# nicolaivicol/otto-recommender

Hardware: AMD Instinct MI355X
Metric: co-visit pairs/sec + candidates/sec at 220M events, 1/2/4/8 MI355X (higher is better)
Workload: dtype int32; 1 GPU; configs[1]: all 5 co-visitation rules, 220M events, 100k-session files; events=220000079, sessions=13435907, parallelism=files dealt over 1 GPU(s)

## Files before the change

### otto-recommender_amd/csrc/abi.hip

```cpp
#include <cstdarg>
#include <cstdlib>
#include <ctime>
#include <algorithm>
#include <mutex>
#include "prims.h"
#include "covis_kernels.h"
#include "table.h"

using namespace ottohip;

namespace ottohip {
static thread_local char g_err[1024] = "";
void set_error(const char* fmt, ...) {
  va_list ap;
  va_start(ap, fmt);
  vsnprintf(g_err, sizeof g_err, fmt, ap);
  va_end(ap);
}
}

namespace ottohip {
Ctx* ctx_base(ottohip_ctx* c) { return c; }

int ensure_part_stats(const ottohip_table* tc) {
// ... 96 lines not shown
  const int dev = it->second.first;
  auto& fr = g_cache[dev].free_;
  fr.emplace(it->second.second, p);
  g_cache_live.erase(it);
  size_t tot = 0;
  for (auto& kv : fr) tot += kv.first;
  if (tot <= cache_cap()) return;
  int prev = -1;
  (void)hipGetDevice(&prev);
  if (prev != dev) (void)hipSetDevice(dev);
  while (tot > cache_cap() && !fr.empty()) {
    auto last = std::prev(fr.end());
    tot -= last->first;
    (void)hipDeviceSynchronize();
    (void)hipFree(last->second);
    fr.erase(last);
  }
  if (prev != dev) (void)hipSetDevice(prev);
}

void dev_trim() {
  std::lock_guard<std::mutex> lk(g_cache_mu);
  auto it = g_cache.find(cur_device());
  if (it == g_cache.end() || it->second.free_.empty()) return;
  (void)hipDeviceSynchronize();
  for (auto& kv : it->second.free_) (void)hipFree(kv.second);
  it->second.free_.clear();
}
}


struct Front {
  RulesDev R;
  Layout Lt;
  int64_t E = 0, Sn = 0, NB = 0;
  int nl = 0;
  const int64_t* off = nullptr;
  int64_t *first = nullptr, *fb = nullptr, *d_loff = nullptr;
  int32_t* long_list = nullptr;
  uint32_t* fid = nullptr;
  uint64_t* evp = nullptr;
  uint64_t* lscr = nullptr;
  uint32_t* lpscr = nullptr;
  uint32_t* cnt = nullptr;
  uint32_t* link = nullptr;
  uint64_t* poff = nullptr;
  uint32_t* poff32 = nullptr;
  uint64_t P = 0;
  int64_t Rn = 0;
  uint32_t* row_key = nullptr;
  uint64_t* row_begin = nullptr;
};

struct KeptEmission {
  uint32_t* words = nullptr;
  uint32_t* row_key = nullptr;
  uint64_t* row_begin = nullptr;
  uint64_t P = 0;
  int64_t Rn = 0;
  RulesDev R;
  Layout Lt;
  int n_rules = 0, n_files = 0;
};
void kept_free(KeptEmission* k) {
  if (!k) return;
  dev_free(k->words);
// ... 71 lines not shown
static ottohip_table* new_table(ottohip_ctx* ctx, int n_rules, int32_t n_items) {
  ottohip_table* T = new ottohip_table();
  T->device = ctx->device;
  T->n_rules = n_rules;
  T->n_items = n_items;
  T->ctx = ctx;
  memset(T->stats, 0, sizeof T->stats);
  return T;
}

static int owner_map(ottohip_ctx* ctx, int32_t n_items, int G, hipStream_t s, const uint32_t** a2l,
                     const uint32_t** l2a, const uint32_t** obase, int* LB) {
  uint32_t *da2l, *dl2a, *dob;
  OH_TRY(ctx->ws.get("om_a2l", (size_t)std::max(n_items, 1), &da2l));
  OH_TRY(ctx->ws.get("om_l2a", (size_t)std::max(n_items, 1), &dl2a));
  OH_TRY(ctx->ws.get("om_obase", (size_t)G + 1, &dob));
  if (ctx->om_items != n_items || ctx->om_parts != G) {
    std::vector<uint32_t> cnt(G + 1, 0), a2l_h(std::max(n_items, 1)), l2a_h(std::max(n_items, 1));
    for (int32_t a = 0; a < n_items; ++a) a2l_h[a] = cnt[owner_dev((uint32_t)a, (uint32_t)G)]++;
    uint32_t mx = 0;
    std::vector<uint32_t> ob(G + 1, 0);
    for (int o = 0; o < G; ++o) { mx = std::max(mx, cnt[o]); ob[o + 1] = ob[o] + cnt[o]; }
    for (int32_t a = 0; a < n_items; ++a) l2a_h[ob[owner_dev((uint32_t)a, (uint32_t)G)] + a2l_h[a]] = (uint32_t)a;
    OH_HIP(hipMemcpyAsync(da2l, a2l_h.data(), (size_t)n_items * 4, hipMemcpyHostToDevice, s));
    OH_HIP(hipMemcpyAsync(dl2a, l2a_h.data(), (size_t)n_items * 4, hipMemcpyHostToDevice, s));
    OH_HIP(hipMemcpyAsync(dob, ob.data(), (size_t)(G + 1) * 4, hipMemcpyHostToDevice, s));
    OH_HIP(hipStreamSynchronize(s));
    ctx->om_items = n_items;
    ctx->om_parts = G;
    ctx->om_lb = std::max(1, bits_for((uint64_t)mx));
  }
  *a2l = da2l; *l2a = dl2a; *obase = dob; *LB = ctx->om_lb;
  return 0;
}

static int covis_front(ottohip_ctx* ctx, const ottohip_events* ev, const ottohip_covis_params* params,
                       const int32_t* file_ids, int n_parts, Front& F, hipStream_t s, ottohip_emit* EM = nullptr) {
  ++ctx->gen;
  const int64_t E = ev->n_events, Sn = ev->n_sessions;
  F.E = E; F.Sn = Sn;
  F.P = 0; F.Rn = 0;
  if (E == 0 || Sn == 0) return 0;
  Workspace& ws = ctx->ws;
  const Layout& Lt = F.Lt;
  const RulesDev& R = F.R;
  const int64_t NB = ceil_div(E, EV_BLOCK);
  F.NB = NB;
  int32_t* n_long;
  int* err;
  const int64_t long_cap = E / (LCAP + 1) + 1;
  OH_TRY(ws.get("first", (size_t)NB + 1, &F.first));
  OH_TRY(ws.get("fb", (size_t)ev->n_files + 1, &F.fb));
  OH_TRY(ws.get("fid", (size_t)ev->n_files, &F.fid));
  OH_TRY(ws.get("long_list", (size_t)long_cap, &F.long_list));
  OH_TRY(ws.get("n_long", 4, &n_long));
  OH_TRY(ws.get("err", 4, &err));
  std::vector<uint32_t> fid(ev->n_files);
  for (int f = 0; f < ev->n_files; ++f) fid[f] = file_ids ? (uint32_t)file_ids[f] : (uint32_t)f;
  OH_HIP(hipMemcpyAsync(F.fb, ev->file_session_bounds, (ev->n_files + 1) * sizeof(int64_t), hipMemcpyHostToDevice, s));
  OH_HIP(hipMemcpyAsync(F.fid, fid.data(), ev->n_files * sizeof(uint32_t), hipMemcpyHostToDevice, s));
  OH_HIP(hipMemsetAsync(n_long, 0, 4 * sizeof(int32_t), s));
  OH_HIP(hipMemsetAsync(err, 0, sizeof(int), s));
  OH_HIP(hipStreamSynchronize(s));
  const int64_t* off = ev->session_offsets;
  F.off = off;

  uint32_t *rk, *pos, *rk2, *pos2;
  OH_TRY(ws.get("ev", (size_t)E, &F.evp));
  OH_TRY(ws.get("cnt", (size_t)E, &F.cnt));
  OH_TRY(ws.get("rk", (size_t)E, &rk));
  OH_TRY(ws.get("pos", (size_t)E, &pos));
  OH_TRY(ws.get("rk2", (size_t)E, &rk2));
  OH_TRY(ws.get("pos2", (size_t)E, &pos2));
  static const bool rows_legacy = getenv("OTTOHIP_ROWS") && !strcmp(getenv("OTTOHIP_ROWS"), "legacy");
  const int cshift = (Lt.A + 2 + 7) / 8 * 8;
  const bool ol_env = !(getenv("OTTOHIP_OWNER_LOCAL") && !strcmp(getenv("OTTOHIP_OWNER_LOCAL"), "0"));
  const uint32_t *om_a2l = nullptr, *om_l2a = nullptr, *om_obase = nullptr;
  int om_lb = 0;
  bool owner_local = false;
  if (!rows_legacy && n_parts > 1 && ol_env && cshift + 8 <= 32 && 3ull * (uint64_t)params->n_items < (1ull << 24)) {
    OH_TRY(owner_map(ctx, params->n_items, n_parts, s, &om_a2l, &om_l2a, &om_obase, &om_lb));
    owner_local = ((uint64_t)n_parts << (om_lb + 2)) < (1ull << cshift);
  }
  const bool fused = !rows_legacy && (n_parts == 1 || owner_local) && cshift + 8 <= 32 &&
                     3ull * (uint64_t)params->n_items < (1ull << 24);
  uint32_t* pos_w = fused ? nullptr : pos;
  static const bool rows_atomic = getenv("OTTOHIP_ROWS") && !strcmp(getenv("OTTOHIP_ROWS"), "atomic");
  const bool group = fused && !rows_atomic && !(getenv("OTTOHIP_GROUP") && !strcmp(getenv("OTTOHIP_GROUP"), "0"));
  F.link = nullptr;
  if (group) OH_TRY(ws.get("link", (size_t)E, &F.link));
  int ph = ctx->begin("prep_count", s, 9.0 * E + 8.0 * (Sn + 1) + 8.0 * E + 12.0 * E);
  k_block_first<<<grid_for(Sn + 1), 256, 0, s>>>(off, Sn, NB, F.first, F.long_list, n_long);
  k_prep_count<<<(unsigned)NB, 64, 0, s>>>(off, F.first, NB, ev->aid, ev->ts, ev->type, F.evp, params->n_items,
                                           params->dedup, err, R, Lt.A, F.cnt, rk, pos_w, fused ? cshift : 0, F.link);
  if (hipGetLastError() != hipSuccess) { set_error("k_prep_count launch failed"); return OTTOHIP_EHIP; }
  int32_t nl = 0;
  OH_TRY(d2h(&nl, n_long, 1, s));
  F.nl = nl;
  if (nl > 0) {
    std::vector<int32_t> ll(nl);
    OH_TRY(d2h(ll.data(), F.long_list, (size_t)nl, s));
    std::sort(ll.begin(), ll.end());
    OH_HIP(hipMemcpy(F.long_list, ll.data(), nl * sizeof(int32_t), hipMemcpyHostToDevice));
    std::vector<int64_t> loff(nl + 1);
    loff[0] = 0;
    for (int i = 0; i < nl; ++i) {
      int64_t ab[2];
      OH_HIP(hipMemcpy(ab, off + ll[i], 2 * sizeof(int64_t), hipMemcpyDeviceToHost));
      loff[i + 1] = loff[i] + (ab[1] - ab[0]);
    }
    OH_TRY(ws.get("long_scr", (size_t)(2 * loff[nl]), &F.lscr));
    OH_TRY(ws.get("long_pscr", (size_t)(3 * (loff[nl] + nl)), &F.lpscr));
    OH_TRY(ws.get("long_off", (size_t)(nl + 1), &F.d_loff));
    OH_HIP(hipMemcpy(F.d_loff, loff.data(), (nl + 1) * sizeof(int64_t), hipMemcpyHostToDevice));
    k_prep_long<<<nl, 64, 0, s>>>(off, F.long_list, F.d_loff, F.lscr, ev->aid, ev->ts, ev->type, F.evp,
                                  params->n_items, params->dedup, err);
    k_count_long<<<nl, 64, 0, s>>>(off, F.long_list, F.d_loff, F.lscr, F.lpscr, F.evp, R, Lt.A, F.cnt, rk, pos_w,
                                   fused ? cshift : 0, F.link);
    if (hipGetLastError() != hipSuccess) { set_error("long-session launch failed"); return OTTOHIP_EHIP; }
  }
  ctx->end(ph, s);

  ph = ctx->begin("rows", s, 0);
  if (rows_atomic && fused) {
    const uint32_t INVa = 3u << Lt.A;
    const uint32_t kmask_a = Lt.A + 2 >= 32 ? ~0u : (1u << (Lt.A + 2)) - 1u;
    const int64_t nk = (int64_t)3 << Lt.A;
// ... 103 lines not shown
  uint64_t *woff, *row_idx;
  OH_TRY(ws.get("woff", (size_t)E, &woff));
  OH_TRY(ws.get("row_idx", (size_t)E, &row_idx));
  OH_TRY(exclusive_scan_u32(ctx, c_sorted, woff, E, tot, s));
  OH_TRY(exclusive_scan_u32(ctx, row_flag, row_idx, E, tot + 1, s));
  uint64_t PR[2];
  OH_TRY(d2h(PR, tot, 2, s));
  int herr = 0;
  OH_TRY(d2h(&herr, err, 1, s));
  if (herr) { set_error("input out of range: aid outside [0, n_items) or type outside {0,1,2}"); return OTTOHIP_ERANGE; }
  F.P = PR[0];
  F.Rn = (int64_t)PR[1];
  OH_TRY(ws.get("poff", (size_t)E, &F.poff));
  F.poff32 = nullptr;
  OH_TRY(ws.get("row_key", (size_t)std::max<int64_t>(F.Rn, 1), &F.row_key));
  OH_TRY(ws.get("row_begin", (size_t)std::max<int64_t>(F.Rn, 1), &F.row_begin));
  k_rows<<<grid_for(E), 256, 0, s>>>(rks, poss, E, INV, kmask, woff, row_flag, row_idx, F.poff, F.row_key,
                                     F.row_begin);
  ctx->end(ph, s);
  return 0;
}

static int covis_emit_words(ottohip_ctx* ctx, const Front& F, const ottohip_events* ev, uint32_t* w0, hipStream_t s) {
  int ph = ctx->begin("emit", s, 8.0 * F.E + 12.0 * F.E + 4.0 * (double)F.P);
  static const int dbg0 = getenv("OTTOHIP_EMIT_DBG") ? atoi(getenv("OTTOHIP_EMIT_DBG")) : 0;
  const int dbg = dbg0;
  const bool guard = getenv("OTTOHIP_DEBUG") != nullptr;
  int* eerr;
  OH_TRY(ctx->ws.get("emit_err", 4, &eerr));
  OH_HIP(hipMemsetAsync(eerr, 0, sizeof(int), s));
  const bool tasks = !(getenv("OTTOHIP_EMIT_TASKS") && !strcmp(getenv("OTTOHIP_EMIT_TASKS"), "0"));
  const bool fl2 = !(getenv("OTTOHIP_EMIT_FLUSH2") && !strcmp(getenv("OTTOHIP_EMIT_FLUSH2"), "0"));
  const bool flq = tasks && fl2 && !(getenv("OTTOHIP_EMIT_FLUSHQ") && !strcmp(getenv("OTTOHIP_EMIT_FLUSHQ"), "0"));
  auto ek = guard ? (tasks ? (flq ? k_emit<true, true, true, EB_Q> : k_emit<true, true, true>) : k_emit<true, false, true>)
                  : (tasks ? (flq ? k_emit<false, true, true, EB_Q> : fl2 ? k_emit<false, true, true> : k_emit<false, true, false>)
                           : k_emit<false, false, true>);
  if (F.NB > 0)
    ek<<<(unsigned)F.NB, 64, 0, s>>>(F.off, F.first, F.NB, F.evp, F.R, F.Lt, F.fb, ev->n_files, F.fid, F.cnt,
                                         EvOff{F.poff, F.poff32, nullptr}, w0, eerr, dbg);
  if (F.nl > 0)
    k_emit_long<<<F.nl, 64, 0, s>>>(F.off, F.long_list, F.d_loff, F.lscr, F.lpscr, F.evp, F.R, F.Lt, F.fb,
                                     ev->n_files, F.fid, F.cnt, EvOff{F.poff, F.poff32, nullptr}, w0);
  if (hipGetLastError() != hipSuccess) { set_error("k_emit launch failed"); return OTTOHIP_EHIP; }
  ctx->end(ph, s);
  int herr = 0;
  OH_TRY(d2h(&herr, eerr, 1, s));
  if (herr & 8) { set_error("emit: record index outside the flush's records (err=%d)", herr); return OTTOHIP_EHIP; }
  if (herr) { set_error("emit: pairs written per event disagree with the count stage (err=%d)", herr); return OTTOHIP_EHIP; }
  return 0;
}

static int file_opts_setup(ottohip_ctx* ctx, const ottohip_file_opts* o, int n_rules, const RulesDev& R,
                           FileOpts& fo, hipStream_t s) {
  if (o->rule < 0 || o->rule >= n_rules) { set_error("file_opts: rule %d outside the call's rules", o->rule); return OTTOHIP_EINVAL; }
  const bool want_hist = o->file_rows || o->file_rows_ge2;
  if (want_hist && (o->n_files < 1 || o->n_files > FO_MAXF)) {
    set_error("file_opts: n_files=%d outside [1, %d]", o->n_files, FO_MAXF); return OTTOHIP_ELIMIT;
  }
  memset(&fo, 0, sizeof fo);
  for (int t = 0; t < 3; ++t)
    for (int q = 0; q < R.n_of_type[t]; ++q)
      if (R.rule_of_type[t][q] == o->rule) { fo.type = t; fo.q = (uint32_t)q; }
  fo.sym = (uint32_t)((R.sym_mask >> o->rule) & 1u);
  if (fo.sym && (o->lo_file >= 0 || o->hi_file >= 0)) { set_error("file_opts: key cuts on a symmetric table"); return OTTOHIP_EINVAL; }
  fo.lo_file = o->lo_file < 0 ? 0xFFFFFFFFu : (uint32_t)o->lo_file;
  fo.hi_file = o->hi_file < 0 ? 0xFFFFFFFFu : (uint32_t)o->hi_file;
  fo.cuts = (o->lo_file >= 0 || o->hi_file >= 0) ? 1u : 0u;
  fo.lo_key = o->lo_key;
  fo.hi_key = o->hi_key;
  OH_TRY(ctx->ws.get("fo_dropped", 1, &fo.dropped));
  OH_HIP(hipMemsetAsync(fo.dropped, 0, 8, s));
  if (getenv("OTTOHIP_DEBUG")) {
// ... 1456 lines not shown
```

### otto-recommender_amd/csrc/covis_kernels.h

```cpp
#pragma once
#include "prims.h"

namespace ottohip {

constexpr int EV_BLOCK = 256;
constexpr int LCAP = 512;
constexpr int SPLIT_MEAN = 420;
constexpr int LDS_SPLIT_MEAN = 2560;
__constant__ uint32_t c_split_mean = SPLIT_MEAN;
__constant__ uint32_t c_split_runs = 0;
__constant__ uint32_t c_split_fuse = 1;
__constant__ uint32_t c_hash_prio = 0;
__constant__ uint32_t c_lds_leaf = 0;
constexpr uint32_t W_EMPTY = 0xFFFFFFFFu;
constexpr int STAT_STRIPES = 256;
constexpr int STAT_RAW = MAX_RULES * 4;
constexpr int STAT_STRIDE = STAT_RAW + 8;

struct RulesDev {
  int32_t lo[MAX_RULES], hi[MAX_RULES];
  uint32_t mask[MAX_RULES];
  int32_t n_of_type[4];
  int32_t rule_of_type[4][MAX_RULES];
  uint32_t sym_mask;
};

__device__ __forceinline__ bool rule_sym(const RulesDev& R, int r) { return (R.sym_mask >> r) & 1u; }

__device__ __forceinline__ uint32_t count_sym_partners(const uint64_t* ev, int jb, int je, uint32_t aid, int t, int A) {
  const uint32_t lo = (aid << 2) | (uint32_t)t;
  uint32_t m = 0;
  if (A > 29) {
    for (int j = jb; j < je; ++j) {
      const uint32_t w = (uint32_t)ev[j];
      m += ((w & 3u) == (uint32_t)t && w >= lo) ? 1u : 0u;
    }
    return m;
  }
  constexpr uint32_t LIM = 1u << 29;
  auto ok = [&](uint32_t w) { return __builtin_amdgcn_alignbit(w - lo, w - lo, 2) < LIM ? 1u : 0u; };
  int j = jb;
  for (; j + 4 <= je; j += 4) m += ok((uint32_t)ev[j]) + ok((uint32_t)ev[j + 1]) + ok((uint32_t)ev[j + 2]) + ok((uint32_t)ev[j + 3]);
  for (; j < je; ++j) m += ok((uint32_t)ev[j]);
  return m;
}

struct Layout {
  int A;
  int F;
  int BR;
  int WB;
  uint32_t amask;
};

struct Task {
  uint64_t begin;
  uint32_t len;
  uint32_t row;
  uint32_t rem;
  uint32_t buf;
// ... 253 lines not shown
                                                   uint32_t* __restrict__ pos, int cshift, uint32_t* __restrict__ link) {
  const int64_t s = list[blockIdx.x];
  const int64_t e0 = off[s];
  const int n = (int)(off[s + 1] - e0);
  const int64_t so = scratch_off[blockIdx.x];
  SessView S;
  uint64_t* evs = scratch + 2 * so;
  uint32_t* pref = pscratch + 3 * (so + blockIdx.x);
  S.ev = evs; S.pref = pref; S.pstride = n + 1;
  S.nv = load_session(ev + e0, n, evs, pref, n + 1);
  count_session(S, e0, n, R, A, cnt, rk, pos, cshift, link);
}

__device__ __forceinline__ int lds_lower_ts(const uint64_t* tev, int a, int b, int64_t x) {
  while (a < b) {
    const int m = (a + b) >> 1;
    if ((int64_t)ev_ts(tev[m]) < x) a = m + 1; else b = m;
  }
  return a;
}
__device__ __forceinline__ int lds_upper_ts(const uint64_t* tev, int a, int b, int64_t x) {
  while (a < b) {
    const int m = (a + b) >> 1;
    if ((int64_t)ev_ts(tev[m]) <= x) a = m + 1; else b = m;
  }
  return a;
}

constexpr int PB_CAP = 512;
struct PrepLds {
  uint64_t key[PB_CAP];
  union {
    uint64_t srt[PB_CAP];
    uint16_t pref[3][PB_CAP + 1];
  };
  uint16_t ss[65];
  uint16_t pst[64], pen[64];
  uint8_t esid[PB_CAP];
  uint8_t uns[64];
};
static_assert((uint64_t)PB_CAP * MAX_RULES * (LCAP - 1) < (1ull << LK_DSHIFT), "group prefixes in link bits");

__global__ __launch_bounds__(64) void k_prep_count(const int64_t* __restrict__ off, const int64_t* __restrict__ first,
                                                   int64_t NB, const int32_t* __restrict__ aid,
                                                   const int32_t* __restrict__ ts, const int8_t* __restrict__ ty,
                                                   uint64_t* __restrict__ ev, int n_items, int dedup, int* err,
                                                   RulesDev R, int A, uint32_t* __restrict__ cnt,
                                                   uint32_t* __restrict__ rk, uint32_t* __restrict__ pos, int cshift,
                                                   uint32_t* __restrict__ link) {
  __shared__ PrepLds S;
  __shared__ RulesDev sR;
  const int l = threadIdx.x;
  if (l == 0) sR = R;
  const int64_t g = blockIdx.x;
  if (g >= NB) return;
  const int64_t s0 = first[g], s1 = first[g + 1];
  __syncthreads();
  const uint32_t INV = 3u << A;
  int64_t b = s0;
  while (b < s1) {
    const int64_t base = off[b];
    const int64_t s = b + l;
    const bool in_s = s < s1;
    const int64_t so = in_s ? off[s] : 0, se = in_s ? off[s + 1] : 0;
    const bool ok = in_s && se - base <= PB_CAP && se - so <= LCAP;
    const uint64_t bad = __ballot(!ok);
    const int nsess = bad ? (int)__builtin_ctzll(bad) : 64;
    if (nsess == 0) { ++b; continue; }
    const int nb_ev = __shfl((int)(se - base), nsess - 1);
    const int64_t E0 = base;
    if (l < nsess) { S.ss[l] = (uint16_t)(so - base); S.uns[l] = 0; }
    if (l == 0) S.ss[nsess] = (uint16_t)nb_ev;
    __builtin_amdgcn_wave_barrier();
    __builtin_amdgcn_fence(__ATOMIC_SEQ_CST, "wavefront");
    const int nch = (nb_ev + 63) >> 6;
#pragma unroll 1
    for (int c = 0; c < nch; ++c) {
      const int idx = c * 64 + l;
      if (idx >= nb_ev) continue;
      const int32_t a = aid[E0 + idx], t = ts[E0 + idx], y = ty[E0 + idx];
      if (a < 0 || a >= n_items || y < 0 || y > 2) atomicOr(err, 1);
      S.key[idx] = ev_pack(a < 0 ? 0 : a, t, y & 3);
      int k = 0;
#pragma unroll
      for (int st = 32; st >= 1; st >>= 1)
        if (k + st < nsess && (int)S.ss[k + st] <= idx) k += st;
// ... 47 lines not shown
      if (in) S.key[idx] = EV_INVALID;
      P += (uint32_t)__popcll(m);
    }
    __builtin_amdgcn_wave_barrier();
    __builtin_amdgcn_fence(__ATOMIC_SEQ_CST, "wavefront");
    P = 0;
#pragma unroll 1
    for (int c = 0; c < nch; ++c) {
      const int idx = c * 64 + l;
      const bool in = idx < nb_ev;
      const int k = in ? S.esid[idx] : 0;
      const bool keep = in && (!dedup || idx == (int)S.ss[k] || S.srt[idx - 1] != S.srt[idx]);
      const uint64_t m = __ballot(keep);
      if (keep) S.key[S.ss[k] + (P + mbcnt(m)) - S.pst[k]] = S.srt[idx];
      P += (uint32_t)__popcll(m);
    }
    __builtin_amdgcn_wave_barrier();
    __builtin_amdgcn_fence(__ATOMIC_SEQ_CST, "wavefront");
    uint32_t b0 = 0, b1 = 0, b2 = 0;
#pragma unroll 1
    for (int c = 0; c < nch; ++c) {
      const int idx = c * 64 + l;
      const bool in = idx < nb_ev;
      const uint64_t v = in ? S.key[idx] : EV_INVALID;
      if (in) ev[E0 + idx] = v;
      const int t = ev_type(v);
      const uint64_t m0 = __ballot(t == 0), m1 = __ballot(t == 1), m2 = __ballot(t == 2);
      if (in) {
        S.pref[0][idx] = (uint16_t)(b0 + mbcnt(m0));
        S.pref[1][idx] = (uint16_t)(b1 + mbcnt(m1));
        S.pref[2][idx] = (uint16_t)(b2 + mbcnt(m2));
      }
      b0 += (uint32_t)__popcll(m0); b1 += (uint32_t)__popcll(m1); b2 += (uint32_t)__popcll(m2);
    }
    if (l == 0) { S.pref[0][nb_ev] = (uint16_t)b0; S.pref[1][nb_ev] = (uint16_t)b1; S.pref[2][nb_ev] = (uint16_t)b2; }
    __builtin_amdgcn_wave_barrier();
    __builtin_amdgcn_fence(__ATOMIC_SEQ_CST, "wavefront");
    constexpr int NCH = PB_CAP / 64;
    uint32_t cv[NCH];
#pragma unroll
    for (int c = 0; c < NCH; ++c) cv[c] = 0u;
#pragma unroll 1
    for (int c = 0; c < nch; ++c) {
      const int idx = c * 64 + l;
      if (idx >= nb_ev) continue;
      const int k = S.esid[idx];
      const uint64_t e = S.key[idx];
      uint32_t cn = 0, key = INV;
      if (e != EV_INVALID) {
        const int lo = S.ss[k], hi = lo + (S.pen[k] - S.pst[k]);
        const int t = ev_type(e);
        const int64_t tsi = ev_ts(e);
        int run = -1;
#if defined(OH_PREP_ABL) && OH_PREP_ABL == 3
        cn = 1;
        if (false)
#endif
        int32_t plo = 1, phi = -1;
        int jb = 0, je = 0;
        for (int q = 0; q < sR.n_of_type[t]; ++q) {
          const int r = sR.rule_of_type[t][q];
          if (sR.lo[r] != plo || sR.hi[r] != phi) {
            plo = sR.lo[r]; phi = sR.hi[r];
            const bool around = plo <= 0 && phi >= 0;
            jb = lds_lower_ts(S.key, lo, around ? idx : hi, tsi + plo);
            je = lds_upper_ts(S.key, around ? idx + 1 : jb, hi, tsi + phi);
          }
          if (je <= jb) continue;
          uint32_t m = 0;
          if (rule_sym(sR, r)) {
#if defined(OH_PREP_ABL) && OH_PREP_ABL == 1
            m = (uint32_t)(je - jb);
#else
            m = count_sym_partners(S.key, jb, je, (uint32_t)ev_aid(e), t, A);
#endif
          } else {
#pragma unroll
            for (int tt = 0; tt < 3; ++tt)
              if ((sR.mask[r] >> tt) & 1u) m += (uint32_t)S.pref[tt][je] - (uint32_t)S.pref[tt][jb];
          }
          if (((sR.mask[r] >> t) & 1u) && sR.lo[r] <= 0 && sR.hi[r] >= 0) {
            if (run < 0) {
              int a = idx, z = idx + 1;
              while (a > lo && S.key[a - 1] == e) --a;
              while (z < hi && S.key[z] == e) ++z;
              run = z - a;
            }
            m -= (uint32_t)run;
          }
          cn += m;
        }
        if (cn) key = ((uint32_t)t << A) | (uint32_t)ev_aid(e);
      }
      cnt[E0 + idx] = cn;
      if (link) {
#pragma unroll
        for (int j = 0; j < NCH; ++j)
          if (j == c) cv[j] = cn;
      } else {
// ... 436 lines not shown
}

constexpr int EB_CAP = 512;
#ifndef OH_EB_RCAP
#define OH_EB_RCAP 64
#endif
#ifndef OH_EMIT_WPE
#define OH_EMIT_WPE
#endif
constexpr int EB_RCAP = OH_EB_RCAP;
static_assert(EB_RCAP >= 64 && EB_RCAP <= 128, "records per emit flush");
constexpr uint32_t EB_NONE = 1023u;

struct EmitRecs {
  uint4 rec[EB_RCAP];
  uint64_t rout[EB_RCAP];
  uint32_t rpre[EB_RCAP];
};
struct EmitPre {
  uint16_t pst[3][64], pen[3][64];
};
struct EmitLds {
  uint64_t tev[EB_CAP];
  union {
    EmitRecs r;
    EmitPre p;
  } u;
  uint16_t ss[65];
  uint16_t sb[4][64];
  uint32_t sfile[64];
  uint16_t espos[EB_CAP];
  uint8_t esid[EB_CAP];
  uint32_t mark[128];
};

template <bool GUARD>
__device__ __forceinline__ void emit_flush(EmitLds& S, int nrec, uint32_t tot, int F, uint32_t* __restrict__ words,
                                           int dbg, uint32_t& rid, int* __restrict__ err) {
  if (dbg & 2) return;
  const uint32_t l = lane_id();
  const uint32_t sa = (int)l < nrec ? S.u.r.rpre[l] : 0xFFFFFFFFu;
  const uint32_t sb = (int)l + 64 < nrec ? S.u.r.rpre[l + 64] : 0xFFFFFFFFu;
  const uint64_t below = (1ull << l) - 1ull, upto = below | (1ull << l);
  int ob = -1;
  uint32_t cc = 0;
  for (uint32_t c = 0; c < tot; c += 64) {
    ++rid;
    if (sa - c < 64u) S.mark[sa - c] = rid;
    if (sb - c < 64u) S.mark[sb - c] = rid;
    __builtin_amdgcn_wave_barrier();
    __builtin_amdgcn_fence(__ATOMIC_SEQ_CST, "wavefront");
    const uint64_t mm = __ballot(S.mark[l] == rid);
    const uint64_t mle = mm & upto;
#ifndef OH_EMIT_NOCHECK
    const int o = min(max(ob + (int)__popcll(mle), 0), nrec - 1);
#else
    const int o = ob + (int)__popcll(mle);
#endif
    ob += (int)__popcll(mm);
    const uint32_t p = c + l;
    bool qual = false;
    uint32_t word = 0;
    const bool bad = GUARD && p < tot && (o < 0 || o >= nrec);
    if (bad) atomicOr(err, 8);
    if (p < tot && !bad) {
      const uint4 rc = S.u.r.rec[o];
// ... 188 lines not shown
  }
#ifndef OH_EMIT_NOCHECK
  if (tot > 0 && ob != nrec - 1 && l == 0) atomicOr(err, 8);
#endif
}

struct EmitTasks {
  uint8_t e[3][3 * MAX_RULES];
  uint8_t n[4];
};
__device__ inline void emit_tasks_build(const RulesDev& R, EmitTasks& T) {
  for (int t = 0; t < 3; ++t) {
    int n = 0;
    for (int pass = 0; pass < 2; ++pass)
      for (int q = 0; q < R.n_of_type[t]; ++q) {
        const int r = R.rule_of_type[t][q];
        if (rule_sym(R, r) != (pass == 1)) continue;
        for (int tt = 0; tt < 3; ++tt)
          if ((R.mask[r] >> tt) & 1u) T.e[t][n++] = (uint8_t)(q | (tt << 4) | (pass << 6));
      }
    T.n[t] = (uint8_t)n;
  }
  T.n[3] = 0;
}

template <bool GUARD, bool FL2, int FQ>
__device__ __forceinline__ void emit_flush_sel(EmitLds& S, int nrec, uint32_t tot, int F, uint32_t* __restrict__ words,
                                               int dbg, uint32_t& rid, int* __restrict__ err) {
  if constexpr (FQ > 0) emit_flushq<FQ, GUARD>(S, nrec, tot, F, words, dbg, rid, err);
  else if constexpr (FL2) emit_flush2<GUARD>(S, nrec, tot, F, words, dbg, rid, err);
  else emit_flush<GUARD>(S, nrec, tot, F, words, dbg, rid, err);
}

template <bool GUARD, bool TASKS, bool FL2 = true, int FQ = 0>
__global__ __launch_bounds__(64) OH_EMIT_WPE void k_emit(const int64_t* __restrict__ off, const int64_t* __restrict__ first,
                                             int64_t NB, const uint64_t* __restrict__ ev, RulesDev R, Layout L,
                                             const int64_t* __restrict__ fb, int nf, const uint32_t* __restrict__ fid,
                                             const uint32_t* __restrict__ cnt, EvOff poff,
                                             uint32_t* __restrict__ words, int* __restrict__ err, int dbg) {
  static_assert(FQ == 0 || TASKS, "emit_flushq records are built by the task-list pass 3");
  __shared__ EmitLds S;
  __shared__ RulesDev sR;
  __shared__ EmitTasks sT;
  const int l = threadIdx.x;
  if (l == 0) sR = R;
  if (TASKS && l == 0) emit_tasks_build(R, sT);
  const int64_t g = blockIdx.x;
  if (g >= NB) return;
  const int64_t s0 = first[g], s1 = first[g + 1];
  if (s0 >= s1) return;
  const int shiftR = L.A + L.F;
  int maxq = 0;
#pragma unroll
  for (int t = 0; t < 3; ++t) maxq = max(maxq, R.n_of_type[t]);
  S.mark[l] = 0u;
  S.mark[64 + l] = 0u;
  uint32_t rid = 0;
  int fcur = file_of(fb, nf, s0);
  int64_t next_b = fcur + 1 < nf ? fb[fcur + 1] : INT64_MAX;
  uint32_t fid_cur = fid[fcur];
  __syncthreads();
  const int maxtask = TASKS ? max((int)sT.n[0], max((int)sT.n[1], (int)sT.n[2])) : 0;

  int64_t b = s0;
  while (b < s1) {
    const int64_t base = off[b];
    const int64_t s = b + l;
    const bool in_s = s < s1;
    const int64_t so = in_s ? off[s] : 0, se = in_s ? off[s + 1] : 0;
    const bool ok = in_s && se - base <= EB_CAP && se - so <= LCAP;
    const uint64_t bad = __ballot(!ok);
    const int nsess = bad ? (int)__builtin_ctzll(bad) : 64;
    if (nsess == 0) { ++b; continue; }
    const int nb_ev = (int)(__shfl((int)(se - base), nsess - 1));
    const int64_t E0 = base;
    if (l < nsess) S.ss[l] = (uint16_t)(so - base);
    if (l == 0) S.ss[nsess] = (uint16_t)nb_ev;
    const int64_t s_last = b + nsess - 1;
    if (s_last < next_b) {
      if (l < nsess) S.sfile[l] = fid_cur;
    } else {
      int fk = fcur;
      if (l < nsess) {
        while (fk + 1 < nf && fb[fk + 1] <= s) ++fk;
        S.sfile[l] = fid[fk];
      }
      fcur = __shfl(fk, nsess - 1);
      next_b = fcur + 1 < nf ? fb[fcur + 1] : INT64_MAX;
      fid_cur = fid[fcur];
    }
    __builtin_amdgcn_wave_barrier();
    __builtin_amdgcn_fence(__ATOMIC_SEQ_CST, "wavefront");

    constexpr int NCH = EB_CAP / 64;
    const int nch = (nb_ev + 63) >> 6;
    uint64_t vv[NCH];
    uint32_t sid[NCH], pr[NCH];
#pragma unroll
    for (int c = 0; c < NCH; ++c) {
      const int idx = c * 64 + l;
      vv[c] = (c < nch && idx < nb_ev) ? ev[E0 + idx] : EV_INVALID;
    }
    uint32_t base0 = 0, base1 = 0, base2 = 0;
#pragma unroll
    for (int c = 0; c < NCH; ++c) {
      if (c >= nch) break;
      const int idx = c * 64 + l;
      const bool in = idx < nb_ev;
      const int t = in ? ev_type(vv[c]) : 3;
      int k = 0;
#pragma unroll
      for (int st = 32; st >= 1; st >>= 1)
        if (k + st < nsess && (int)S.ss[k + st] <= idx) k += st;
      const uint64_t m0 = __ballot(t == 0), m1 = __ballot(t == 1), m2 = __ballot(t == 2);
      const uint32_t P0 = base0 + mbcnt(m0), P1 = base1 + mbcnt(m1), P2 = base2 + mbcnt(m2);
      if (in && idx == (int)S.ss[k]) { S.u.p.pst[0][k] = P0; S.u.p.pst[1][k] = P1; S.u.p.pst[2][k] = P2; }
      if (in && idx == (int)S.ss[k + 1] - 1) {
        S.u.p.pen[0][k] = P0 + (t == 0); S.u.p.pen[1][k] = P1 + (t == 1); S.u.p.pen[2][k] = P2 + (t == 2);
      }
      base0 += (uint32_t)__popcll(m0); base1 += (uint32_t)__popcll(m1); base2 += (uint32_t)__popcll(m2);
      sid[c] = (uint32_t)k;
      pr[c] = t == 0 ? P0 : (t == 1 ? P1 : P2);
    }
    __builtin_amdgcn_wave_barrier();
    __builtin_amdgcn_fence(__ATOMIC_SEQ_CST, "wavefront");
    if (l < nsess) {
      const uint32_t a = S.ss[l];
      if (S.ss[l + 1] > a) {
        const uint32_t c0 = S.u.p.pen[0][l] - S.u.p.pst[0][l], c1 = S.u.p.pen[1][l] - S.u.p.pst[1][l], c2 = S.u.p.pen[2][l] - S.u.p.pst[2][l];
        S.sb[0][l] = a; S.sb[1][l] = a + c0; S.sb[2][l] = a + c0 + c1; S.sb[3][l] = a + c0 + c1 + c2;
      }
    }
    __builtin_amdgcn_wave_barrier();
    __builtin_amdgcn_fence(__ATOMIC_SEQ_CST, "wavefront");
#pragma unroll
    for (int c = 0; c < NCH; ++c) {
      if (c >= nch) break;
      const int idx = c * 64 + l;
      const int t = ev_type(vv[c]);
      if (idx < nb_ev) {
        uint32_t pos = EB_NONE;
        if (t < 3) {
          const uint32_t k = sid[c];
          pos = S.sb[t][k] + pr[c] - S.u.p.pst[t][k];
          S.tev[pos] = vv[c];
        }
        S.espos[idx] = (uint16_t)pos;
        S.esid[idx] = (uint8_t)sid[c];
      }
    }
    __builtin_amdgcn_wave_barrier();
    __builtin_amdgcn_fence(__ATOMIC_SEQ_CST, "wavefront");
    int nrec = 0;
    uint32_t tot = 0;
#pragma unroll 1
    for (int c = 0; c < nch; ++c) {
      const int idx = c * 64 + l;
      const bool in = idx < nb_ev;
      const uint32_t sp = in ? S.espos[idx] : EB_NONE;
      const bool valid = sp != EB_NONE;
      const uint64_t v = valid ? S.tev[sp] : EV_INVALID;
      const int t = ev_type(v);
      const uint32_t k = in ? S.esid[idx] : 0u;
      const uint64_t eout = valid && cnt[E0 + idx] ? poff.run(E0 + idx) : 0;
      const uint32_t ecnt = valid ? cnt[E0 + idx] : 0;
      const int64_t tsi = ev_ts(v);
      const uint32_t file = S.sfile[k];
      uint32_t rlo = sp, rhi = sp + 1;
      if (valid) {
        const uint32_t lb = S.sb[t][k], ub = S.sb[t + 1][k];
        while (rlo > lb && S.tev[rlo - 1] == v) --rlo;
        while (rhi < ub && S.tev[rhi] == v) ++rhi;
      }
      uint32_t eo = 0;
      bool has_sym = false;
      if constexpr (TASKS) {
        const int ntk = valid ? (int)sT.n[t] : 0;
#pragma unroll 1
        for (int kk = 0; kk < maxtask; ++kk) {
          const bool act = kk < ntk;
          if (!__ballot(act)) break;
          const uint32_t te = act ? (uint32_t)sT.e[t][kk] : 0u;
          const int q = (int)(te & 15u), tt = (int)((te >> 4) & 3u);
          const bool sym = act && ((te >> 6) & 1u);
          const int r = act ? sR.rule_of_type[t][q] : 0;
          const int32_t lo = sR.lo[r], hi = sR.hi[r];
          has_sym |= sym;
          uint32_t len = 0, jb = 0, xlo = EB_NONE, xlen = 0;
          if (act) {
            const int a = S.sb[tt][k], e = S.sb[tt + 1][k];
            const bool own = tt == t && lo <= 0 && hi >= 0;
            jb = (uint32_t)lds_lower_ts(S.tev, a, own ? (int)rlo : e, tsi + lo);
            const uint32_t je = (uint32_t)lds_upper_ts(S.tev, own ? (int)rhi : (int)jb, e, tsi + hi);
            len = je - jb;
            if (own) { xlo = rlo; xlen = rhi - rlo; len -= xlen; }
            if (FQ > 0 && sym && ecnt == eo) len = 0;
          }
          const uint64_t m = __ballot(len > 0);
          const int nn = (int)__popcll(m);
          if (nn == 0) continue;
          if (nrec + nn > EB_RCAP) {
            __builtin_amdgcn_wave_barrier();
            __builtin_amdgcn_fence(__ATOMIC_SEQ_CST, "wavefront");
            emit_flush_sel<GUARD, FL2, FQ>(S, nrec, tot, L.F, words, dbg, rid, err);
            __builtin_amdgcn_wave_barrier();
            __builtin_amdgcn_fence(__ATOMIC_SEQ_CST, "wavefront");
            nrec = 0; tot = 0;
          }
          constexpr uint32_t GQ = FQ > 0 ? (uint32_t)FQ : 1u;
          const uint32_t units = (len + GQ - 1u) / GQ;
          const uint32_t incl = wave_incl_scan(units);
          if (GUARD && nrec + nn > EB_RCAP) atomicOr(err, 8);
          if (len > 0 && !(GUARD && nrec + (int)mbcnt(m) >= EB_RCAP)) {
            const int ri = nrec + (int)mbcnt(m);
            S.u.r.rpre[ri] = tot + incl - units;
            S.u.r.rec[ri] = make_uint4(FQ > 0 ? len : tot + incl - units, jb | (xlo << 10) | (xlen << 21), ((uint32_t)q << shiftR) | file,
                                   sym ? (uint32_t)ev_aid(v) : 0u);
            S.u.r.rout[ri] = eout + eo;
          }
          if (!sym) eo += len;
          nrec += nn;
          tot += __shfl(incl, 63);
        }
      } else {
        const int nq = valid ? sR.n_of_type[t] : 0;
        bool lane_sym = false;
        for (int q = 0; q < nq; ++q) lane_sym |= rule_sym(sR, sR.rule_of_type[t][q]);
        const int nqq = __ballot(lane_sym) ? 2 * maxq : maxq;
#pragma unroll 1
        for (int qq = 0; qq < nqq; ++qq) {
          const int q = qq % maxq, pass = qq / maxq;
          const int r = q < nq ? sR.rule_of_type[t][q] : 0;
          const bool sym = q < nq && rule_sym(sR, r);
          const uint32_t msk = (q < nq && sym == (pass == 1)) ? sR.mask[r] : 0u;
          const int32_t lo = sR.lo[r], hi = sR.hi[r];
          has_sym |= msk != 0u && sym;
#pragma unroll 1
          for (int tt = 0; tt < 3; ++tt) {
            const bool act = (msk >> tt) & 1u;
            if (!__ballot(act)) continue;
// ... 2026 lines not shown
```

Baseline: 84.63 billion pairs/s.

## Narrow time-window binary searches using precomputed gap-segment bitmasks

Adds per-window gap segmentation. Ballot bitmasks mark session edges and time gaps larger than each window radius. Prep_count, and emit when WIN_SEG bit 2 is set, use these segment bounds to narrow the LDS binary searches. When a whole segment spans no more than the smaller window side, the search is skipped entirely. Emit needs extra LDS state (type masks, bases, session offsets) and must recompute registers after a flush. This adds ballot, readlane and shared-memory overhead and increases LDS use, which may lower occupancy. By default only the prep_count path is enabled (WIN_SEG_DEFAULT=1).

```diff
diff --git a/otto-recommender_amd/csrc/abi.hip b/otto-recommender_amd/csrc/abi.hip
--- a/otto-recommender_amd/csrc/abi.hip
+++ b/otto-recommender_amd/csrc/abi.hip
@@ -152,6 +152,7 @@
 
 struct Front {
   RulesDev R;
+  WinSeg W{}, We{};
   Layout Lt;
   int64_t E = 0, Sn = 0, NB = 0;
   int nl = 0;
@@ -289,6 +290,33 @@
   }
   *a2l = da2l; *l2a = dl2a; *obase = dob; *LB = ctx->om_lb;
   return 0;
+}
+
+constexpr int WIN_SEG_DEFAULT = 1;
+static WinSeg win_seg_build(const RulesDev& R, bool on, int max_win = WS_MAX) {
+  WinSeg W;
+  memset(&W, 0, sizeof W);
+  int32_t wlo[WS_MAX], whi[WS_MAX];
+  for (int r = 0; r < MAX_RULES; ++r) W.of_rule[r] = -1;
+  if (!on) return W;
+  for (int t = 0; t < 3; ++t)
+    for (int q = 0; q < R.n_of_type[t]; ++q) {
+      const int r = R.rule_of_type[t][q];
+      const int32_t lo = R.lo[r], hi = R.hi[r];
+      if (!(lo <= 0 && hi >= 0)) continue;
+      int w = 0;
+      while (w < W.n && (wlo[w] != lo || whi[w] != hi)) ++w;
+      if (w == max_win) continue;
+      if (w == W.n) {
+        const uint32_t below = (uint32_t)(-(int64_t)lo), above = (uint32_t)hi;
+        wlo[w] = lo; whi[w] = hi;
+        W.gap[w] = std::max(below, above);
+        W.span[w] = std::min(below, above);
+        ++W.n;
+      }
+      W.of_rule[r] = (int8_t)w;
+    }
+  return W;
 }
 
 static int covis_front(ottohip_ctx* ctx, const ottohip_events* ev, const ottohip_covis_params* params,
@@ -346,10 +374,14 @@
   const bool group = fused && !rows_atomic && !(getenv("OTTOHIP_GROUP") && !strcmp(getenv("OTTOHIP_GROUP"), "0"));
   F.link = nullptr;
   if (group) OH_TRY(ws.get("link", (size_t)E, &F.link));
+  const int wseg = getenv("OTTOHIP_WIN_SEG") ? atoi(getenv("OTTOHIP_WIN_SEG")) : WIN_SEG_DEFAULT;
+  F.W = win_seg_build(R, (wseg & 1) != 0);
+  F.We = win_seg_build(R, (wseg & 2) != 0, WS_EMIT);
   int ph = ctx->begin("prep_count", s, 9.0 * E + 8.0 * (Sn + 1) + 8.0 * E + 12.0 * E);
   k_block_first<<<grid_for(Sn + 1), 256, 0, s>>>(off, Sn, NB, F.first, F.long_list, n_long);
   k_prep_count<<<(unsigned)NB, 64, 0, s>>>(off, F.first, NB, ev->aid, ev->ts, ev->type, F.evp, params->n_items,
-                                           params->dedup, err, R, Lt.A, F.cnt, rk, pos_w, fused ? cshift : 0, F.link);
+                                           params->dedup, err, R, Lt.A, F.cnt, rk, pos_w, fused ? cshift : 0, F.link,
+                                           F.W);
   if (hipGetLastError() != hipSuccess) { set_error("k_prep_count launch failed"); return OTTOHIP_EHIP; }
   int32_t nl = 0;
   OH_TRY(d2h(&nl, n_long, 1, s));
@@ -519,12 +551,15 @@
   const bool tasks = !(getenv("OTTOHIP_EMIT_TASKS") && !strcmp(getenv("OTTOHIP_EMIT_TASKS"), "0"));
   const bool fl2 = !(getenv("OTTOHIP_EMIT_FLUSH2") && !strcmp(getenv("OTTOHIP_EMIT_FLUSH2"), "0"));
   const bool flq = tasks && fl2 && !(getenv("OTTOHIP_EMIT_FLUSHQ") && !strcmp(getenv("OTTOHIP_EMIT_FLUSHQ"), "0"));
-  auto ek = guard ? (tasks ? (flq ? k_emit<true, true, true, EB_Q> : k_emit<true, true, true>) : k_emit<true, false, true>)
-                  : (tasks ? (flq ? k_emit<false, true, true, EB_Q> : fl2 ? k_emit<false, true, true> : k_emit<false, true, false>)
+  const bool seg = flq && F.We.n > 0;
+  auto ek = guard ? (tasks ? (flq ? (seg ? k_emit<true, true, true, EB_Q, true> : k_emit<true, true, true, EB_Q>) : k_emit<true, true, true>)
+                           : k_emit<true, false, true>)
+                  : (tasks ? (flq ? (seg ? k_emit<false, true, true, EB_Q, true> : k_emit<false, true, true, EB_Q>)
+                                  : fl2 ? k_emit<false, true, true> : k_emit<false, true, false>)
                            : k_emit<false, false, true>);
   if (F.NB > 0)
     ek<<<(unsigned)F.NB, 64, 0, s>>>(F.off, F.first, F.NB, F.evp, F.R, F.Lt, F.fb, ev->n_files, F.fid, F.cnt,
-                                         EvOff{F.poff, F.poff32, nullptr}, w0, eerr, dbg);
+                                         EvOff{F.poff, F.poff32, nullptr}, w0, eerr, dbg, F.We);
   if (F.nl > 0)
     k_emit_long<<<F.nl, 64, 0, s>>>(F.off, F.long_list, F.d_loff, F.lscr, F.lpscr, F.evp, F.R, F.Lt, F.fb,
                                      ev->n_files, F.fid, F.cnt, EvOff{F.poff, F.poff32, nullptr}, w0);
diff --git a/otto-recommender_amd/csrc/covis_kernels.h b/otto-recommender_amd/csrc/covis_kernels.h
--- a/otto-recommender_amd/csrc/covis_kernels.h
+++ b/otto-recommender_amd/csrc/covis_kernels.h
@@ -26,6 +26,38 @@
 };
 
 __device__ __forceinline__ bool rule_sym(const RulesDev& R, int r) { return (R.sym_mask >> r) & 1u; }
+
+constexpr int WS_MAX = 4;
+constexpr int WS_EMIT = 2;
+struct WinSeg {
+  uint32_t gap[WS_MAX];
+  uint32_t span[WS_MAX];
+  int8_t of_rule[MAX_RULES];
+  int32_t n;
+};
+__device__ __forceinline__ uint32_t seg_bounds(const uint64_t* bm, int c, int nch, int nb_ev) {
+  const int l = (int)lane_id();
+  const uint64_t mj = bm[l & 7];
+  const uint32_t has = (uint32_t)__ballot(l < nch && mj != 0);
+  const uint32_t mlo = (uint32_t)mj, mhi = (uint32_t)(mj >> 32);
+  auto word = [&](int j) {
+    return ((uint64_t)(uint32_t)__builtin_amdgcn_readlane((int)mhi, j) << 32) | (uint32_t)__builtin_amdgcn_readlane((int)mlo, j);
+  };
+  const uint64_t cur = word(c);
+  const uint32_t before = has & ((1u << c) - 1u), after = has & ~((2u << c) - 1u);
+  int pv = 0, nx = nb_ev;
+  if (before) { const int j = 31 - __builtin_clz(before); pv = j * 64 + 63 - __builtin_clzll(word(j)); }
+  if (after) { const int j = __builtin_ctz(after); nx = j * 64 + __builtin_ctzll(word(j)); }
+  const uint64_t le = (2ull << l) - 1ull;
+  const uint64_t ml = cur & le, mh = cur & ~le;
+  const int A = ml ? c * 64 + 63 - __builtin_clzll(ml) : pv;
+  const int Z = mh ? c * 64 + __builtin_ctzll(mh) : nx;
+  return (uint32_t)A | ((uint32_t)Z << 10);
+}
+static_assert(WS_MAX == 4, "one uint4 member per window");
+__device__ __forceinline__ uint32_t seg_pick(const uint4& sg, int w) {
+  return w == 0 ? sg.x : (w == 1 ? sg.y : (w == 2 ? sg.z : sg.w));
+}
 
 __device__ __forceinline__ uint32_t count_sym_partners(const uint64_t* ev, int jb, int je, uint32_t aid, int t, int A) {
   const uint32_t lo = (aid << 2) | (uint32_t)t;
@@ -345,7 +377,11 @@
   uint64_t key[PB_CAP];
   union {
     uint64_t srt[PB_CAP];
-    uint16_t pref[3][PB_CAP + 1];
+    struct {
+      uint16_t pref[3][PB_CAP + 1];
+      uint16_t pad_;
+      uint64_t bmask[WS_MAX][PB_CAP / 64];
+    };
   };
   uint16_t ss[65];
   uint16_t pst[64], pen[64];
@@ -353,6 +389,7 @@
   uint8_t uns[64];
 };
 static_assert((uint64_t)PB_CAP * MAX_RULES * (LCAP - 1) < (1ull << LK_DSHIFT), "group prefixes in link bits");
+static_assert(offsetof(PrepLds, ss) == 2 * PB_CAP * 8, "the breakpoint words fit the slack of the srt / pref union");
 
 __global__ __launch_bounds__(64) void k_prep_count(const int64_t* __restrict__ off, const int64_t* __restrict__ first,
                                                    int64_t NB, const int32_t* __restrict__ aid,
@@ -360,11 +397,12 @@
                                                    uint64_t* __restrict__ ev, int n_items, int dedup, int* err,
                                                    RulesDev R, int A, uint32_t* __restrict__ cnt,
                                                    uint32_t* __restrict__ rk, uint32_t* __restrict__ pos, int cshift,
-                                                   uint32_t* __restrict__ link) {
+                                                   uint32_t* __restrict__ link, WinSeg W) {
   __shared__ PrepLds S;
   __shared__ RulesDev sR;
+  __shared__ WinSeg sW;
   const int l = threadIdx.x;
-  if (l == 0) sR = R;
+  if (l == 0) { sR = R; sW = W; }
   const int64_t g = blockIdx.x;
   if (g >= NB) return;
   const int64_t s0 = first[g], s1 = first[g + 1];
@@ -478,6 +516,17 @@
         S.pref[2][idx] = (uint16_t)(b2 + mbcnt(m2));
       }
       b0 += (uint32_t)__popcll(m0); b1 += (uint32_t)__popcll(m1); b2 += (uint32_t)__popcll(m2);
+      if (sW.n > 0) {
+        const uint32_t hw = (uint32_t)(v >> 32), k = in ? (uint32_t)S.esid[idx] : 0x100u;
+        uint32_t hp = lane_prev(hw), kp = lane_prev(k);
+        if (l == 0) { hp = c ? (uint32_t)(S.key[idx - 1] >> 32) : hw; kp = c ? (uint32_t)S.esid[idx - 1] : 0x200u; }
+        const bool edge = in && (k != kp || v == EV_INVALID);
+        const uint32_t gap = hw - hp;
+        for (int w = 0; w < sW.n; ++w) {
+          const uint64_t bm = __ballot(edge || (in && gap > sW.gap[w]));
+          if (l == 0) S.bmask[w][c] = bm;
+        }
+      }
     }
     if (l == 0) { S.pref[0][nb_ev] = (uint16_t)b0; S.pref[1][nb_ev] = (uint16_t)b1; S.pref[2][nb_ev] = (uint16_t)b2; }
     __builtin_amdgcn_wave_barrier();
@@ -489,6 +538,13 @@
 #pragma unroll 1
     for (int c = 0; c < nch; ++c) {
       const int idx = c * 64 + l;
+      auto seg_of = [&](int w) -> uint32_t {
+        if (w >= sW.n) return 0u;
+        const uint32_t az = seg_bounds(S.bmask[w], c, nch, nb_ev);
+        const uint32_t ha = (uint32_t)(S.key[az & 1023u] >> 32), hz = (uint32_t)(S.key[(az >> 10) - 1u] >> 32);
+        return az | (hz - ha <= sW.span[w] ? 1u << 20 : 0u);
+      };
+      const uint4 sg = make_uint4(seg_of(0), seg_of(1), seg_of(2), seg_of(3));
       if (idx >= nb_ev) continue;
       const int k = S.esid[idx];
       const uint64_t e = S.key[idx];
@@ -498,19 +554,28 @@
         const int t = ev_type(e);
         const int64_t tsi = ev_ts(e);
         int run = -1;
+        int32_t plo = 1, phi = -1;
+        int jb = 0, je = 0;
 #if defined(OH_PREP_ABL) && OH_PREP_ABL == 3
         cn = 1;
         if (false)
 #endif
-        int32_t plo = 1, phi = -1;
-        int jb = 0, je = 0;
         for (int q = 0; q < sR.n_of_type[t]; ++q) {
           const int r = sR.rule_of_type[t][q];
           if (sR.lo[r] != plo || sR.hi[r] != phi) {
             plo = sR.lo[r]; phi = sR.hi[r];
             const bool around = plo <= 0 && phi >= 0;
-            jb = lds_lower_ts(S.key, lo, around ? idx : hi, tsi + plo);
-            je = lds_upper_ts(S.key, around ? idx + 1 : jb, hi, tsi + phi);
+            const int w = sW.of_rule[r];
+            if (w >= 0) {
+              const uint32_t g = seg_pick(sg, w);
+              const int A = (int)(g & 1023u), Z = (int)((g >> 10) & 1023u);
+              const bool fast = (g >> 20) != 0u;
+              jb = lds_lower_ts(S.key, A, fast ? A : idx, tsi + plo);
+              je = lds_upper_ts(S.key, fast ? Z : idx + 1, Z, tsi + phi);
+            } else {
+              jb = lds_lower_ts(S.key, lo, around ? idx : hi, tsi + plo);
+              je = lds_upper_ts(S.key, around ? idx + 1 : jb, hi, tsi + phi);
+            }
           }
           if (je <= jb) continue;
           uint32_t m = 0;
@@ -1013,6 +1078,12 @@
   uint16_t espos[EB_CAP];
   uint8_t esid[EB_CAP];
   uint32_t mark[128];
+};
+struct EmitSegLds {
+  uint64_t tmask[3][EB_CAP / 64 + 1];
+  uint64_t bmask[WS_EMIT][EB_CAP / 64];
+  uint16_t tbase[3][EB_CAP / 64 + 1];
+  uint16_t soff[3][64];
 };
 
 template <bool GUARD>
@@ -1267,18 +1338,22 @@
   else emit_flush<GUARD>(S, nrec, tot, F, words, dbg, rid, err);
 }
 
-template <bool GUARD, bool TASKS, bool FL2 = true, int FQ = 0>
+template <bool GUARD, bool TASKS, bool FL2 = true, int FQ = 0, bool SEG = false>
 __global__ __launch_bounds__(64) OH_EMIT_WPE void k_emit(const int64_t* __restrict__ off, const int64_t* __restrict__ first,
                                              int64_t NB, const uint64_t* __restrict__ ev, RulesDev R, Layout L,
                                              const int64_t* __restrict__ fb, int nf, const uint32_t* __restrict__ fid,
                                              const uint32_t* __restrict__ cnt, EvOff poff,
-                                             uint32_t* __restrict__ words, int* __restrict__ err, int dbg) {
+                                             uint32_t* __restrict__ words, int* __restrict__ err, int dbg, WinSeg W) {
   static_assert(FQ == 0 || TASKS, "emit_flushq records are built by the task-list pass 3");
+  static_assert(!SEG || FQ > 0, "gap segments: the task-list pass 3 with emit_flushq");
   __shared__ EmitLds S;
+  __shared__ EmitSegLds G;
   __shared__ RulesDev sR;
   __shared__ EmitTasks sT;
+  __shared__ WinSeg sW;
   const int l = threadIdx.x;
   if (l == 0) sR = R;
+  if (SEG && l == 0) sW = W;
   if (TASKS && l == 0) emit_tasks_build(R, sT);
   const int64_t g = blockIdx.x;
   if (g >= NB) return;
@@ -1337,6 +1412,7 @@
       vv[c] = (c < nch && idx < nb_ev) ? ev[E0 + idx] : EV_INVALID;
     }
     uint32_t base0 = 0, base1 = 0, base2 = 0;
+    uint32_t hlast = 0u, klast = 0x200u;
 #pragma unroll
     for (int c = 0; c < NCH; ++c) {
       if (c >= nch) break;
@@ -1353,9 +1429,32 @@
       if (in && idx == (int)S.ss[k + 1] - 1) {
         S.u.p.pen[0][k] = P0 + (t == 0); S.u.p.pen[1][k] = P1 + (t == 1); S.u.p.pen[2][k] = P2 + (t == 2);
       }
+      if constexpr (SEG) {
+        if (sW.n > 0) {
+          if (l == 0) {
+            G.tmask[0][c] = m0; G.tmask[1][c] = m1; G.tmask[2][c] = m2;
+            G.tbase[0][c] = (uint16_t)base0; G.tbase[1][c] = (uint16_t)base1; G.tbase[2][c] = (uint16_t)base2;
+          }
+          const uint32_t hw = (uint32_t)(vv[c] >> 32), kk = in ? (uint32_t)k : 0x100u;
+          uint32_t hp = lane_prev(hw), kp = lane_prev(kk);
+          if (l == 0) { hp = hlast; kp = klast; }
+          hlast = (uint32_t)__builtin_amdgcn_readlane((int)hw, 63);
+          klast = (uint32_t)__builtin_amdgcn_readlane((int)kk, 63);
+          const bool edge = in && (kk != kp || vv[c] == EV_INVALID);
+          const uint32_t gap = hw - hp;
+          for (int w = 0; w < sW.n; ++w) {
+            const uint64_t bm = __ballot(edge || (in && gap > sW.gap[w]));
+            if (l == 0) G.bmask[w][c] = bm;
+          }
+        }
+      }
       base0 += (uint32_t)__popcll(m0); base1 += (uint32_t)__popcll(m1); base2 += (uint32_t)__popcll(m2);
       sid[c] = (uint32_t)k;
       pr[c] = t == 0 ? P0 : (t == 1 ? P1 : P2);
+    }
+    if (SEG && l == 0 && sW.n > 0) {
+      G.tmask[0][nch] = 0ull; G.tmask[1][nch] = 0ull; G.tmask[2][nch] = 0ull;
+      G.tbase[0][nch] = (uint16_t)base0; G.tbase[1][nch] = (uint16_t)base1; G.tbase[2][nch] = (uint16_t)base2;
     }
     __builtin_amdgcn_wave_barrier();
     __builtin_amdgcn_fence(__ATOMIC_SEQ_CST, "wavefront");
@@ -1364,6 +1463,11 @@
       if (S.ss[l + 1] > a) {
         const uint32_t c0 = S.u.p.pen[0][l] - S.u.p.pst[0][l], c1 = S.u.p.pen[1][l] - S.u.p.pst[1][l], c2 = S.u.p.pen[2][l] - S.u.p.pst[2][l];
         S.sb[0][l] = a; S.sb[1][l] = a + c0; S.sb[2][l] = a + c0 + c1; S.sb[3][l] = a + c0 + c1 + c2;
+        if constexpr (SEG) {
+          G.soff[0][l] = (uint16_t)(a - S.u.p.pst[0][l]);
+          G.soff[1][l] = (uint16_t)(a + c0 - S.u.p.pst[1][l]);
+          G.soff[2][l] = (uint16_t)(a + c0 + c1 - S.u.p.pst[2][l]);
+        }
       }
     }
     __builtin_amdgcn_wave_barrier();
@@ -1394,13 +1498,13 @@
       const bool in = idx < nb_ev;
       const uint32_t sp = in ? S.espos[idx] : EB_NONE;
       const bool valid = sp != EB_NONE;
-      const uint64_t v = valid ? S.tev[sp] : EV_INVALID;
-      const int t = ev_type(v);
-      const uint32_t k = in ? S.esid[idx] : 0u;
+      uint64_t v = valid ? S.tev[sp] : EV_INVALID;
+      int t = ev_type(v);
+      uint32_t k = in ? S.esid[idx] : 0u;
       const uint64_t eout = valid && cnt[E0 + idx] ? poff.run(E0 + idx) : 0;
       const uint32_t ecnt = valid ? cnt[E0 + idx] : 0;
-      const int64_t tsi = ev_ts(v);
-      const uint32_t file = S.sfile[k];
+      int64_t tsi = ev_ts(v);
+      uint32_t file = S.sfile[k];
       uint32_t rlo = sp, rhi = sp + 1;
       if (valid) {
         const uint32_t lb = S.sb[t][k], ub = S.sb[t + 1][k];
@@ -1409,8 +1513,21 @@
       }
       uint32_t eo = 0;
       bool has_sym = false;
+      uint2 sg = make_uint2(0u, 0u);
+      auto seg_of = [&](int w) -> uint32_t {
+        if (w >= sW.n) return 0u;
+        const uint32_t az = seg_bounds(G.bmask[w], c, nch, nb_ev);
+        uint32_t f = 0u;
+        if (valid) {
+          const uint32_t ha = (uint32_t)(S.tev[S.espos[az & 1023u]] >> 32);
+          const uint32_t hz = (uint32_t)(S.tev[S.espos[(az >> 10) - 1u]] >> 32);
+          f = hz - ha <= sW.span[w] ? 1u << 20 : 0u;
+        }
+        return az | f;
+      };
+      if constexpr (SEG) sg = make_uint2(seg_of(0), seg_of(1));
       if constexpr (TASKS) {
-        const int ntk = valid ? (int)sT.n[t] : 0;
+        int ntk = valid ? (int)sT.n[t] : 0;
 #pragma unroll 1
         for (int kk = 0; kk < maxtask; ++kk) {
           const bool act = kk < ntk;
@@ -1425,8 +1542,21 @@
           if (act) {
             const int a = S.sb[tt][k], e = S.sb[tt + 1][k];
             const bool own = tt == t && lo <= 0 && hi >= 0;
-            jb = (uint32_t)lds_lower_ts(S.tev, a, own ? (int)rlo : e, tsi + lo);
-            const uint32_t je = (uint32_t)lds_upper_ts(S.tev, own ? (int)rhi : (int)jb, e, tsi + hi);
+            const int w = SEG ? (int)sW.of_rule[r] : -1;
+            uint32_t je;
+            if (SEG && w >= 0) {
+              const uint32_t g = w == 0 ? sg.x : sg.y, so = G.soff[tt][k];
+              auto lpos = [&](uint32_t p) {
+                return so + G.tbase[tt][p >> 6] + (uint32_t)__popcll(G.tmask[tt][p >> 6] & ((1ull << (p & 63u)) - 1ull));
+              };
+              const int pa = (int)lpos(g & 1023u), pz = (int)lpos((g >> 10) & 1023u);
+              const bool fast = (g >> 20) != 0u;
+              jb = (uint32_t)lds_lower_ts(S.tev, pa, fast ? pa : (own ? (int)rlo : pz), tsi + lo);
+              je = (uint32_t)lds_upper_ts(S.tev, fast ? pz : (own ? (int)rhi : (int)jb), pz, tsi + hi);
+            } else {
+              jb = (uint32_t)lds_lower_ts(S.tev, a, own ? (int)rlo : e, tsi + lo);
+              je = (uint32_t)lds_upper_ts(S.tev, own ? (int)rhi : (int)jb, e, tsi + hi);
+            }
             len = je - jb;
             if (own) { xlo = rlo; xlen = rhi - rlo; len -= xlen; }
             if (FQ > 0 && sym && ecnt == eo) len = 0;
@@ -1441,6 +1571,15 @@
             __builtin_amdgcn_wave_barrier();
             __builtin_amdgcn_fence(__ATOMIC_SEQ_CST, "wavefront");
             nrec = 0; tot = 0;
+            if constexpr (SEG) {
+              sg = make_uint2(seg_of(0), seg_of(1));
+              v = valid ? S.tev[sp] : EV_INVALID;
+              t = ev_type(v);
+              tsi = ev_ts(v);
+              k = in ? S.esid[idx] : 0u;
+              file = S.sfile[k];
+              ntk = valid ? (int)sT.n[t] : 0;
+            }
           }
           constexpr uint32_t GQ = FQ > 0 ? (uint32_t)FQ : 1u;
           const uint32_t units = (len + GQ - 1u) / GQ;
```

Result: no change. 84.53 billion pairs/s (-0.1%).
